# bababyVN/medical-image-segmentation-and-classification

Measured on AMD Instinct MI355X. Metric: images/sec (train step) Attention U-Net 256x256 bs=32/GPU, higher is better.
Workload: dtype bf16; 1 GPU; AttentionUNet 256x256 train step (fwd+BCE+bwd+clip+AdamW), bs=32/GPU, NHWC bf16 activations, fp32 master weights; global_batch=32, parallelism=dp1, hip_graph=False, wgrad_side_stream=True, plan_replay=C (mi355_plan_run)

## Files before the change

include/mi355conv.h:

```cpp
#ifndef MI355CONV_H_
#define MI355CONV_H_

#include <stdint.h>

#ifdef __cplusplus
extern "C" {
#endif

typedef struct ihipStream_t* mi355_stream_t;

enum { MI355_F32 = 0, MI355_BF16 = 1, MI355_F16 = 2 };
enum { MI355_OK = 0, MI355_ERR_ARG = -1, MI355_ERR_UNSUPPORTED = -2, MI355_ERR_RUNTIME = -3 };

int mi355_version(void);
const char* mi355_last_error(void);


int mi355_pack_input_nchw(const float* x, void* y, int N, int C, int H, int W, int Cpad, int dtype,
                          mi355_stream_t s);
int mi355_pack_input_im2col3(const float* x, void* y, int N, int C, int H, int W, int dtype, mi355_stream_t s);
int mi355_unpack_output_nchw(const void* x, float* y, int N, int C, int H, int W, int ld, int dtype,
                             mi355_stream_t s);
int mi355_pack_nchw(const float* x, void* y, int N, int C, int H, int W, int ld, int dtype, mi355_stream_t s);

int mi355_pack_conv_weight(const float* w, void* wf, void* wb, int Co, int Ci, int Cip, int KH, int KW,
                           int transposed, int dtype, mi355_stream_t s);

int mi355_pack_conv_weights_batched(const int64_t* table, int n, int fields ,
                                    int dtype, mi355_stream_t s);

int mi355_conv2d_igemm(const void* in, const void* wk, const float* bias, void* out,
                       int N, int Hi, int Wi, int Ci, int ldi,
                       int Ho, int Wo, int Co, int ldo,
                       int KH, int KW, int mul, int kmul, int off, int div, int up,
                       int accumulate, float* stats, int dtype, mi355_stream_t s);
int mi355_conv2d_igemm_variant(int Hi, int Wi, int Ci, int Ho, int Wo, int Co, int KH, int KW, int mul, int kmul, int off,
                               int div, int up, int dtype);
int mi355_conv2d_igemm_variant_n(int N, int Hi, int Wi, int Ci, int Ho, int Wo, int Co, int KH, int KW, int mul, int kmul,
                                 int off, int div, int up, int dtype);
int mi355_conv2d_igemm_dma_tile(int N, int Ho, int Wo, int Ci, int Co);
int mi355_conv2d_igemm_generic_tile(int N, int Ho, int Wo, int Co);
int mi355_conv2d_igemm_stat_rows(int N, int Hi, int Wi, int Ci, int Ho, int Wo, int Co, int KH, int KW,
                                 int mul, int kmul, int off, int div, int up, int dtype);

int mi355_conv2d_wgrad_splits(int N, int Ho, int Wo, int Ci, int Co, int KH, int KW);
int mi355_conv2d_wgrad_variant(int N, int Ho, int Wo, int KH, int KW, int stride, int pad, int dtype);
int mi355_conv2d_wgrad(const void* x, const void* dy, float* ws, int splits,
                       int N, int Hi, int Wi, int Ci, int ldx,
                       int Ho, int Wo, int Co, int ldy,
                       int KH, int KW, int stride, int pad, int up, int dtype, mi355_stream_t s);
int mi355_conv2d_wgrad_multi_ok(int N, int Ho, int Wo, int dtype);
int mi355_conv2d_wgrad_multi(const void* x0, const void* dy0, const void* x1, const void* dy1, const void* x2, const void* dy2,
                             const void* x3, const void* dy3, const void* x4, const void* dy4, const void* x5, const void* dy5,
                             int napp, float* ws, int splits, int N, int Hi, int Wi, int Ci, int ldx, int Ho, int Wo, int Co,
                             int ldy, int up, int dtype, mi355_stream_t s);
int mi355_conv2d_wgrad_reduce(const float* ws, int splits, float* dw, int Co, int Ci, int Ci_real,
                              int KH, int KW, int transposed, float beta, mi355_stream_t s);


int mi355_rowreduce_blocks(long long M);
int mi355_bn_stats(const void* x, float* partial, long long M, int C, int ld, int dtype, mi355_stream_t s);
int mi355_bn_finalize(const float* partial, int nblocks, long long M, int C, const float* gamma,
                      const float* beta, float* running_mean, float* running_var, int64_t* nbt,
                      float momentum, float eps, float* scale, float* shift, float* mean, float* invstd,
                      mi355_stream_t s);
int mi355_fold_rows(const float* partial, int rows, int rowlen, float* out, int nsplit, mi355_stream_t s);
int mi355_bn_fold_bias(const float* bias, const float* scale, const float* shift, float* out, int C, mi355_stream_t s);
int mi355_bn_eval_coeffs(const float* gamma, const float* beta, const float* running_mean,
                         const float* running_var, float eps, int C, float* scale, float* shift,
                         mi355_stream_t s);
int mi355_bn_act(const void* x, int ldx, const float* scale, const float* shift,
                 const void* x2, int ldx2, const float* scale2, const float* shift2,
                 const void* res, int ldr, void* y, int ldy, long long M, int C, int act, int dtype,
                 mi355_stream_t s);
int mi355_bn_act_pool2(const void* x, int ldx, const float* scale, const float* shift, void* y, int ldy, void* p, int ldp,
                       int N, int H, int W, int C, int act, int dtype, mi355_stream_t s);
int mi355_bn_act_windows(const void* x, int ldx, const float* scale, const float* shift, const void* res, int ldr, void* y, int ldy,
                         int N, int H, int W, int C, int act, int dtype, mi355_stream_t s);
int mi355_bn_bwd_reduce_rows(long long M);
int mi355_bn_bwd_reduce(const void* dy, int lddy, const void* y, int ldy, const void* x, int ldx,
                        const float* mean, const float* invstd, const float* mscale, const float* mshift,
                        float* partial, long long M, int C, int act, int dtype, mi355_stream_t s);
int mi355_bn_bwd_finalize(const float* partial, int nblocks, int C, float* sums, float* dgamma, float* dbeta,
                          float acc, mi355_stream_t s);
int mi355_bn_bwd_finalize_at(const float* partial, int nblocks, int nq, int q0, int q1, int C, float* sums, float* dgamma,
                             float* dbeta, float acc, mi355_stream_t s);
int mi355_bn_bwd_apply(const void* dy, int lddy, const void* y, int ldy, const void* x, int ldx,
                       const float* gamma, const float* mean, const float* invstd, const float* mscale,
                       const float* mshift, const float* sums, void* dx, int lddx, void* dres, int lddres,
                       void* dpost, int lddpost, int post_acc, float* dbias_partial,
                       long long M, int C, int act, int dtype, mi355_stream_t s);
int mi355_bn_bwd_apply_post4(const void* dy, int lddy, const void* y, int ldy, const void* x, int ldx,
                             const float* gamma, const float* mean, const float* invstd, const float* mscale,
                             const float* mshift, const float* sums, void* dx, int lddx, void* dpost, int lddpost,
                             int post_acc, const void* ex0, const void* ex1, const void* ex2, const void* ex3, int ldex,
                             long long M, int C, int act, int dtype, mi355_stream_t s);
int mi355_bn_bwd_pool2_ok(int H, int W, int C, int dtype);
int mi355_bn_bwd_reduce_pool2_rows(long long M);
int mi355_bn_bwd_reduce_pool2(const void* dy, int lddy, const void* dp, int lddp, const void* x, int ldx, const float* mean,
                              const float* invstd, const float* mscale, const float* mshift, float* partial,
                              int N, int H, int W, int C, int dtype, mi355_stream_t s);
int mi355_bn_bwd_apply_pool2(const void* dy, int lddy, const void* dp, int lddp, const void* x, int ldx, const float* gamma,
                             const float* mean, const float* invstd, const float* mscale, const float* mshift,
                             const float* sums, void* dx, int lddx, int N, int H, int W, int C, int dtype, mi355_stream_t s);
int mi355_colsum_finalize(const float* partial, int nblocks, int stride, int C, float* out, float acc,
                          mi355_stream_t s);
int mi355_colsum(const void* x, int ld, float* partial, long long M, int C, int dtype, mi355_stream_t s);

int mi355_maxpool_fwd(const void* x, int ldx, void* y, int ldy, int N, int H, int W, int C,
                      int k, int stride, int pad, int dtype, mi355_stream_t s);
int mi355_maxpool_bwd(const void* x, int ldx, const void* dy, int lddy, void* dx, int lddx,
                      int N, int H, int W, int C, int k, int stride, int pad, int accumulate, int dtype,
                      mi355_stream_t s);
int mi355_upsample2_bwd(const void* dy, int lddy, void* dx, int lddx, int N, int H, int W, int C,
                        int accumulate, int dtype, mi355_stream_t s);
int mi355_add(const void* a, int lda, const void* b, int ldb, void* y, int ldy, long long M, int C, int dtype,
              mi355_stream_t s);
int mi355_relu_fwd(const void* x, int ldx, void* y, int ldy, long long M, int C, int dtype, mi355_stream_t s);
int mi355_relu_bwd(const void* dy, int lddy, const void* y, int ldy, void* dx, int lddx, long long M, int C,
                   int dtype, mi355_stream_t s);

int mi355_rowdot_fwd(const void* x, int ldx, const float* w, const float* b, float* z, float* partial,
                     long long M, int C, int HW, int K, int dtype, mi355_stream_t s);
int mi355_rowdot_bwd(const float* dz, const void* x, int ldx, const float* w, void* dx, int lddx,
                     float* partial, long long M, int C, int relu_mask, int HW, int K, int accumulate, int dtype,
                     mi355_stream_t s);
int mi355_gate_mul_fwd(const void* x, int ldx, const float* z, const float* scale, const float* shift,
                       void* y, int ldy, long long M, int C, int dtype, mi355_stream_t s);
int mi355_gate_mul_bwd(const void* dy, int lddy, const void* x, int ldx, const float* z, const float* scale,
// ... 103 lines not shown
```

medical-image-segmentation-and-classification_amd/csrc/conv_wgrad.hip:

```cpp
#include "common.hpp"
#include "dma.hpp"
#include "wgrad3x3_halo.hpp"
#include "wgrad3x3_halo8.hpp"
#include <stdlib.h>

struct WgradArgs {
  const void* x;
  const void* dy;
  float* ws;
  int N, Hi, Wi, Ci, ldx;
  int Ho, Wo, Co, ldy;
  int KH, KW, stride, pad, up;
  int M, Hlog, Wlog;
  int chunk;
};

typedef __attribute__((address_space(3))) s16x4 lds_s16x4;
template <typename T> struct TwoByte { typedef T type; };
template <> struct TwoByte<float> { typedef bf16_t type; };

template <typename T, int BCO, int BCI>
__global__ __launch_bounds__(256) void conv_wgrad_kernel(const WgradArgs a) {
  constexpr int BP = 32;
  constexpr int EPC = 16 / (int)sizeof(T);
  constexpr bool BF = sizeof(T) == 2;
  constexpr int PO = BF ? (BCO == 128 ? 320 : 192) : BCO * 4;
  constexpr int PX = BF ? (BCI == 128 ? 320 : 192) : BCI * 4;
  constexpr int O_BYTES = BP * PO, X_BYTES = BP * PX, STAGE = O_BYTES + X_BYTES;
  constexpr int CPRO = BCO / EPC, CPRX = BCI / EPC;
  constexpr int O_IT = BP * CPRO / 256, X_IT = BP * CPRX / 256;
  constexpr int WTO = BCO / 2, WTI = BCI / 2;
  constexpr int MI = WTO / 32, NI = WTI / 32;
  static_assert(O_IT >= 1 && X_IT >= 1, "tile too small for 256 threads");
  __shared__ __attribute__((aligned(16))) unsigned char lds[2 * STAGE];

  const int tid = threadIdx.x, lane = tid & 63, wave = tid >> 6;
  const int r32 = lane & 31, h = lane >> 5;
  const int wo_ = wave >> 1, wi_ = wave & 1;
  const int ciTiles = (a.Ci + BCI - 1) / BCI;
  int bid = xcd_tile((blockIdx.z * gridDim.y + blockIdx.y) * gridDim.x + blockIdx.x, gridDim.x * gridDim.y * gridDim.z);
  const int bx = bid % gridDim.x; bid /= gridDim.x;
  const int co0 = (bx / ciTiles) * BCO, ci0 = (bx % ciTiles) * BCI;
  const int tap = bid % gridDim.y, kh = tap / a.KW, kw = tap - kh * a.KW;
  const int split = bid / gridDim.y;
  const int p_begin = split * a.chunk;
  const int p_end = min(a.M, p_begin + a.chunk);
  const T* __restrict__ x = reinterpret_cast<const T*>(a.x);
  const T* __restrict__ dy = reinterpret_cast<const T*>(a.dy);

  int o_row[O_IT], o_c[O_IT];
#pragma unroll
  for (int i = 0; i < O_IT; ++i) {
    const int id = tid + i * 256;
    o_row[i] = id / CPRO;
    o_c[i] = id - o_row[i] * CPRO;
  }
  int x_row[X_IT], x_c[X_IT], x_n[X_IT], x_ho[X_IT], x_wo[X_IT];
  const int HoWo = a.Ho * a.Wo;
#pragma unroll
  for (int i = 0; i < X_IT; ++i) {
    const int id = tid + i * 256;
    x_row[i] = id / CPRX;
    x_c[i] = id - x_row[i] * CPRX;
    const int m = p_begin + x_row[i];
    x_n[i] = m / HoWo;
    const int rem = m - x_n[i] * HoWo;
    x_ho[i] = rem / a.Wo;
    x_wo[i] = rem - x_ho[i] * a.Wo;
  }

  uint4 ro[O_IT], rx[X_IT];
  auto load_tile = [&](int p0) {
#pragma unroll
    for (int i = 0; i < O_IT; ++i) {
      const int m = p0 + o_row[i];
      const int c = co0 + o_c[i] * EPC;
      if (m < p_end && c < a.Co)
        ro[i] = *reinterpret_cast<const uint4*>(dy + (size_t)m * a.ldy + c);
      else
        ro[i] = make_uint4(0, 0, 0, 0);
    }
#pragma unroll
    for (int i = 0; i < X_IT; ++i) {
      const int m = p0 + x_row[i];
      const int c = ci0 + x_c[i] * EPC;
      int th = x_ho[i] * a.stride + kh - a.pad, tw = x_wo[i] * a.stride + kw - a.pad;
      bool ok = m < p_end && c < a.Ci && (unsigned)th < (unsigned)a.Hlog && (unsigned)tw < (unsigned)a.Wlog;
// ... 25 lines not shown
  f32x16 acc[MI][NI];
#pragma unroll
  for (int mi = 0; mi < MI; ++mi)
#pragma unroll
    for (int ni = 0; ni < NI; ++ni)
#pragma unroll
      for (int r = 0; r < 16; ++r) acc[mi][ni][r] = 0.f;

  const int steps = (p_end - p_begin + BP - 1) / BP;
  if (steps > 0) {
    load_tile(p_begin);
    store_tile(0);
  }
  __syncthreads();
  const int tq = (lane & 15) >> 2, tp = lane & 3, tg = (lane >> 4) & 1;
  for (int st = 0; st < steps; ++st) {
    const int cur = st & 1;
    const bool more = (st + 1) < steps;
    if (more) load_tile(p_begin + (st + 1) * BP);
    const unsigned char* lo = lds + cur * STAGE;
    const unsigned char* lx = lo + O_BYTES;
    if constexpr (BF) {
#pragma unroll
      for (int ss = 0; ss < 2; ++ss) {
        bf16x8 af[MI], bfr[NI];
#pragma unroll
        for (int mi = 0; mi < MI; ++mi) {
          const int col = wo_ * WTO + mi * 32 + 16 * tg + 4 * tp;
          const int prow = ss * 16 + 8 * h + tq;
          const s16x4 v0 = __builtin_amdgcn_ds_read_tr16_b64_v4i16((lds_s16x4*)(lo + prow * PO + col * 2));
          const s16x4 v1 = __builtin_amdgcn_ds_read_tr16_b64_v4i16((lds_s16x4*)(lo + (prow + 4) * PO + col * 2));
          af[mi] = __builtin_bit_cast(bf16x8, __builtin_shufflevector(v0, v1, 0, 1, 2, 3, 4, 5, 6, 7));
        }
#pragma unroll
        for (int ni = 0; ni < NI; ++ni) {
          const int col = wi_ * WTI + ni * 32 + 16 * tg + 4 * tp;
          const int prow = ss * 16 + 8 * h + tq;
          const s16x4 v0 = __builtin_amdgcn_ds_read_tr16_b64_v4i16((lds_s16x4*)(lx + prow * PX + col * 2));
          const s16x4 v1 = __builtin_amdgcn_ds_read_tr16_b64_v4i16((lds_s16x4*)(lx + (prow + 4) * PX + col * 2));
          bfr[ni] = __builtin_bit_cast(bf16x8, __builtin_shufflevector(v0, v1, 0, 1, 2, 3, 4, 5, 6, 7));
        }
#pragma unroll
        for (int mi = 0; mi < MI; ++mi)
#pragma unroll
          for (int ni = 0; ni < NI; ++ni)
            acc[mi][ni] = mfma_32x32x16<typename TwoByte<T>::type>(af[mi], bfr[ni], acc[mi][ni]);
      }
    } else {
#pragma unroll 4
      for (int s2 = 0; s2 < BP / 2; ++s2) {
        const int prow = 2 * s2 + h;
        float af[MI], bfr[NI];
#pragma unroll
        for (int mi = 0; mi < MI; ++mi)
          af[mi] = *reinterpret_cast<const float*>(lo + prow * PO + (wo_ * WTO + mi * 32 + r32) * 4);
#pragma unroll
        for (int ni = 0; ni < NI; ++ni)
          bfr[ni] = *reinterpret_cast<const float*>(lx + prow * PX + (wi_ * WTI + ni * 32 + r32) * 4);
#pragma unroll
        for (int mi = 0; mi < MI; ++mi)
#pragma unroll
          for (int ni = 0; ni < NI; ++ni)
            acc[mi][ni] = __builtin_amdgcn_mfma_f32_32x32x2f32(af[mi], bfr[ni], acc[mi][ni], 0, 0, 0);
      }
    }
    if (more) store_tile(cur ^ 1);
    __syncthreads();
  }

  const int taps = a.KH * a.KW;
  float* __restrict__ ws = a.ws + (size_t)split * a.Co * taps * a.Ci;
#pragma unroll
  for (int mi = 0; mi < MI; ++mi)
#pragma unroll
    for (int ni = 0; ni < NI; ++ni)
#pragma unroll
      for (int r = 0; r < 16; ++r) {
        const int co = co0 + wo_ * WTO + mi * 32 + (r & 3) + 8 * (r >> 2) + 4 * h;
        const int ci = ci0 + wi_ * WTI + ni * 32 + r32;
        if (co < a.Co && ci < a.Ci) ws[((size_t)co * taps + tap) * a.Ci + ci] = acc[mi][ni][r];
      }
}

static void wgrad_tiles(int Co, int Ci, int& bco, int& bci) {
  bco = (Co % 128 == 0) ? 128 : 64;
  bci = (Ci % 128 == 0) ? 128 : 64;
}

static int halo_wgrad_mode(int N, int Ho, int Wo, int KH, int KW) {
  static const int use8 = getenv("MI355_WGRAD8") ? atoi(getenv("MI355_WGRAD8")) : 1;
  if (KH != 3 || KW != 3 || Ho % 8 != 0) return 0;
  if (use8 && Wo % 64 == 0) return 3;
  if (use8 && Wo == 32 && N % 2 == 0) return 4;
  if (Wo % 32 == 0) return 1;
  if (Wo == 16 && N % 2 == 0) return 2;
  return 0;
}
static int halo_wgrad_items(int mode, int N, int Ho, int Wo, int rb) {
  switch (mode) {
    case 1: return N * (Wo / 32) * (Ho / rb);
    case 3: return N * (Wo / 64) * (Ho / rb);
    default: return (N / 2) * (Ho / rb);
  }
}

extern "C" int mi355_conv2d_wgrad_splits(int N, int Ho, int Wo, int Ci, int Co, int KH, int KW) {
  if (const int mode = halo_wgrad_mode(N, Ho, Wo, KH, KW)) {
    const int rb = Ho % 32 == 0 ? 32 : (Ho % 16 == 0 ? 16 : 8);
    const long long items = halo_wgrad_items(mode, N, Ho, Wo, rb);
    const long long tiles = (long long)ceil_div(Co, 64) * ceil_div(Ci, 64);
    static const int wgs_env = getenv("MI355_WGRAD_WGS") ? atoi(getenv("MI355_WGRAD_WGS")) : 0;
    int wgs = wgs_env > 0 ? wgs_env : (mode >= 3 ? 128 : 256);
    static const int deep_wgs = getenv("MI355_WGRAD_WGS_DEEP") ? atoi(getenv("MI355_WGRAD_WGS_DEEP")) : 0;
    static const int deep_h = getenv("MI355_WGRAD_DEEP_H") ? atoi(getenv("MI355_WGRAD_DEEP_H")) : 64;
    if (mode >= 3 && deep_wgs > 0 && Ho <= deep_h) wgs = deep_wgs;
    long long s = wgs / tiles;
    if (s > items) s = items;
    const long long slab = (long long)Co * 9 * Ci * 4;
    while (s > 1 && s * slab > (512ll << 20)) --s;
    return (int)(s < 1 ? 1 : s);
  }
  int bco, bci;
  wgrad_tiles(Co, Ci, bco, bci);
  const long long M = (long long)N * Ho * Wo;
  const long long tiles = (long long)ceil_div(Co, bco) * ceil_div(Ci, bci) * KH * KW;
  long long s = 768 / tiles;
  const long long max_by_pixels = M / 256 > 0 ? M / 256 : 1;
  if (s > max_by_pixels) s = max_by_pixels;
  const long long slab = (long long)Co * KH * KW * Ci * 4;
  while (s > 1 && s * slab > (512ll << 20)) --s;
  if (s < 1) s = 1;
  return (int)s;
}

template <typename T>
static int wgrad_launch(const WgradArgs& a, int splits, hipStream_t s) {
  int bco, bci;
  wgrad_tiles(a.Co, a.Ci, bco, bci);
  dim3 grid(ceil_div(a.Co, bco) * ceil_div(a.Ci, bci), a.KH * a.KW, splits);
  if (bco == 128 && bci == 128)
    hipLaunchKernelGGL((conv_wgrad_kernel<T, 128, 128>), grid, dim3(256), 0, s, a);
  else if (bco == 128)
    hipLaunchKernelGGL((conv_wgrad_kernel<T, 128, 64>), grid, dim3(256), 0, s, a);
  else if (bci == 128)
    hipLaunchKernelGGL((conv_wgrad_kernel<T, 64, 128>), grid, dim3(256), 0, s, a);
  else
    hipLaunchKernelGGL((conv_wgrad_kernel<T, 64, 64>), grid, dim3(256), 0, s, a);
  MI355_LAUNCH_CHECK();
  return MI355_OK;
}

template <typename T, bool W16>
static int launch_wgrad3x3(const Wgrad3Args& h, dim3 grid, hipStream_t s) {
  constexpr int lds_bytes = Wgrad3Lds<W16>::BYTES;
  static const hipError_t configured =
      hipFuncSetAttribute((const void*)wgrad3x3_halo_kernel<T, W16>, hipFuncAttributeMaxDynamicSharedMemorySize, lds_bytes);
  if (configured != hipSuccess)
    MI355_FAIL((int)configured, "wgrad3x3_halo: cannot reserve %d B of LDS: %s", lds_bytes, hipGetErrorString(configured));
  hipLaunchKernelGGL((wgrad3x3_halo_kernel<T, W16>), grid, dim3(256), lds_bytes, s, h);
  MI355_LAUNCH_CHECK();
  return MI355_OK;
}
template <typename T, bool W32>
static int launch_wgrad3x3_8(const Wgrad3Args& h, dim3 grid, hipStream_t s) {
  constexpr int lds_bytes = Wgrad8Lds::BYTES;
  static const hipError_t configured =
      hipFuncSetAttribute((const void*)wgrad3x3_halo8_kernel<T, W32>, hipFuncAttributeMaxDynamicSharedMemorySize, lds_bytes);
  if (configured != hipSuccess)
    MI355_FAIL((int)configured, "wgrad3x3_halo8: cannot reserve %d B of LDS: %s", lds_bytes, hipGetErrorString(configured));
  hipLaunchKernelGGL((wgrad3x3_halo8_kernel<T, W32>), grid, dim3(512), lds_bytes, s, h);
  MI355_LAUNCH_CHECK();
  return MI355_OK;
}
static int launch_wgrad3x3_any(const Wgrad3Args& h, dim3 grid, int hmode, int dtype, hipStream_t s) {
  const bool f16 = dtype == MI355_F16;
  switch (hmode) {
    case 2: return f16 ? launch_wgrad3x3<f16_t, true>(h, grid, s) : launch_wgrad3x3<bf16_t, true>(h, grid, s);
    case 3: return f16 ? launch_wgrad3x3_8<f16_t, false>(h, grid, s) : launch_wgrad3x3_8<bf16_t, false>(h, grid, s);
    case 4: return f16 ? launch_wgrad3x3_8<f16_t, true>(h, grid, s) : launch_wgrad3x3_8<bf16_t, true>(h, grid, s);
    default: return f16 ? launch_wgrad3x3<f16_t, false>(h, grid, s) : launch_wgrad3x3<bf16_t, false>(h, grid, s);
  }
}

extern "C" int mi355_conv2d_wgrad(const void* x, const void* dy, float* ws, int splits, int N, int Hi, int Wi, int Ci,
                                  int ldx, int Ho, int Wo, int Co, int ldy, int KH, int KW, int stride, int pad, int up,
                                  int dtype, mi355_stream_t s) {
  MI355_CHECK_ARG(x && dy && ws, "conv2d_wgrad: null pointer");
  MI355_CHECK_ARG(splits >= 1 && splits <= 65535, "conv2d_wgrad: splits=%d out of range", splits);
  const int esz = dtype_is_2byte(dtype) ? 2 : 4;
  const int epc = 16 / esz;
  MI355_CHECK_ARG(Ci % epc == 0 && Co % epc == 0, "conv2d_wgrad: Ci=%d / Co=%d must be multiples of %d", Ci, Co, epc);
  MI355_CHECK_ARG(((uintptr_t)x % 16) == 0 && ((uintptr_t)dy % 16) == 0 && (ldx * esz) % 16 == 0 && (ldy * esz) % 16 == 0,
                  "conv2d_wgrad: pointers / channel strides must be 16-byte aligned");
  MI355_CHECK_ARG((long long)N * Ho * Wo < (1ll << 31) && (long long)N * Hi * Wi < (1ll << 31),
                  "conv2d_wgrad: pixel count overflows int32");
  WgradArgs a;
  a.x = x; a.dy = dy; a.ws = ws;
  a.N = N; a.Hi = Hi; a.Wi = Wi; a.Ci = Ci; a.ldx = ldx;
  a.Ho = Ho; a.Wo = Wo; a.Co = Co; a.ldy = ldy;
  a.KH = KH; a.KW = KW; a.stride = stride; a.pad = pad; a.up = up ? 1 : 0;
  a.M = N * Ho * Wo;
  a.Hlog = up ? 2 * Hi : Hi;
  a.Wlog = up ? 2 * Wi : Wi;
  a.chunk = ceil_div(ceil_div(a.M, splits), 32) * 32;
  static const int use_halo = getenv("MI355_WGRAD_HALO") ? atoi(getenv("MI355_WGRAD_HALO")) : 1;
  const int hmode = halo_wgrad_mode(N, Ho, Wo, KH, KW);
  const long long img_lim = (1ll << 31) / (hmode == 2 || hmode == 4 ? 2 : 1);
  const bool fits = (long long)Hi * Wi * ldx * esz < img_lim && (long long)Ho * Wo * ldy * esz < img_lim;
  if (dtype_is_2byte(dtype) && use_halo && stride == 1 && pad == 1 && hmode && Ho == a.Hlog && Wo == a.Wlog && fits) {
    Wgrad3Args h;
    for (int i = 0; i < 6; ++i) { h.xs[i] = x; h.dys[i] = dy; }
    h.ws = ws;
    h.N = N; h.Hi = Hi; h.Wi = Wi; h.Ci = Ci; h.ldx = ldx;
    h.H = Ho; h.W = Wo; h.Co = Co; h.ldy = ldy; h.up = up ? 1 : 0;
    h.RB = Ho % 32 == 0 ? 32 : (Ho % 16 == 0 ? 16 : 8);
    h.items = halo_wgrad_items(hmode, N, Ho, Wo, h.RB);
    h.items_per_app = h.items;
    h.items_per_block = ceil_div(h.items, splits);
    dim3 grid(ceil_div(Co, 64) * ceil_div(Ci, 64), splits);
    return launch_wgrad3x3_any(h, grid, hmode, dtype, (hipStream_t)s);
  }
  return dispatch_dtype(dtype, "conv2d_wgrad", [&](auto tag) { return wgrad_launch<decltype(tag)>(a, splits, (hipStream_t)s); });
}

extern "C" int mi355_conv2d_wgrad_variant(int N, int Ho, int Wo, int KH, int KW, int stride, int pad, int dtype) {
  static const int use_halo = getenv("MI355_WGRAD_HALO") ? atoi(getenv("MI355_WGRAD_HALO")) : 1;
  if (!use_halo || !dtype_is_2byte(dtype) || stride != 1 || pad != 1) return 0;
  return halo_wgrad_mode(N, Ho, Wo, KH, KW);
}

extern "C" int mi355_conv2d_wgrad_multi_ok(int N, int Ho, int Wo, int dtype) {
  static const int use_halo = getenv("MI355_WGRAD_HALO") ? atoi(getenv("MI355_WGRAD_HALO")) : 1;
  return (use_halo && dtype_is_2byte(dtype) && halo_wgrad_mode(N, Ho, Wo, 3, 3)) ? 1 : 0;
}

extern "C" int mi355_conv2d_wgrad_multi(const void* x0, const void* dy0, const void* x1, const void* dy1, const void* x2,
                                        const void* dy2, const void* x3, const void* dy3, const void* x4, const void* dy4,
                                        const void* x5, const void* dy5, int napp, float* ws, int splits, int N, int Hi, int Wi,
                                        int Ci, int ldx, int Ho, int Wo, int Co, int ldy, int up, int dtype, mi355_stream_t s) {
  const void* xs[6] = {x0, x1, x2, x3, x4, x5};
  const void* dys[6] = {dy0, dy1, dy2, dy3, dy4, dy5};
  MI355_CHECK_ARG(napp >= 1 && napp <= 6 && ws && splits >= 1, "conv2d_wgrad_multi: 1..6 operand pairs, a workspace, splits >= 1");
  for (int i = 0; i < napp; ++i)
    MI355_CHECK_ARG(xs[i] && dys[i] && ((uintptr_t)xs[i] % 16) == 0 && ((uintptr_t)dys[i] % 16) == 0,
                    "conv2d_wgrad_multi: pair %d: null or misaligned pointer", i);
  MI355_CHECK_ARG(mi355_conv2d_wgrad_multi_ok(N, Ho, Wo, dtype), "conv2d_wgrad_multi: shape / dtype not served by the nine-tap kernel "
                  "(mi355_conv2d_wgrad_multi_ok == 0): run mi355_conv2d_wgrad per pair");
  MI355_CHECK_ARG(Ci % 8 == 0 && Co % 8 == 0 && (ldx * 2) % 16 == 0 && (ldy * 2) % 16 == 0 && ldx >= Ci && ldy >= Co,
                  "conv2d_wgrad_multi: channel counts / strides must be multiples of 8 elements");
  MI355_CHECK_ARG((up ? (Ho == 2 * Hi && Wo == 2 * Wi) : (Ho == Hi && Wo == Wi)), "conv2d_wgrad_multi: 3x3 / stride 1 / pad 1 geometry only");
  MI355_CHECK_ARG((long long)Hi * Wi * ldx * 4 < (1ll << 31) && (long long)Ho * Wo * ldy * 4 < (1ll << 31),
                  "conv2d_wgrad_multi: an image of 1 GiB or more is beyond the 32-bit offsets of the nine-tap kernel's buffer descriptors");
  const int hmode = halo_wgrad_mode(N, Ho, Wo, 3, 3);
  Wgrad3Args h;
  for (int i = 0; i < 6; ++i) { h.xs[i] = xs[i < napp ? i : 0]; h.dys[i] = dys[i < napp ? i : 0]; }
  h.ws = ws;
  h.N = N; h.Hi = Hi; h.Wi = Wi; h.Ci = Ci; h.ldx = ldx;
  h.H = Ho; h.W = Wo; h.Co = Co; h.ldy = ldy; h.up = up ? 1 : 0;
  h.RB = Ho % 32 == 0 ? 32 : (Ho % 16 == 0 ? 16 : 8);
  h.items_per_app = halo_wgrad_items(hmode, N, Ho, Wo, h.RB);
  h.items = napp * h.items_per_app;
  MI355_CHECK_ARG(splits <= h.items, "conv2d_wgrad_multi: more splits (%d) than work items (%d)", splits, h.items);
  h.items_per_block = ceil_div(h.items, splits);
  dim3 grid(ceil_div(Co, 64) * ceil_div(Ci, 64), splits);
  return launch_wgrad3x3_any(h, grid, hmode, dtype, (hipStream_t)s);
}


#define WR_CI 32
template <int TAPS>
__global__ __launch_bounds__(1024) void wgrad_reduce_kernel(const float* __restrict__ ws, int splits, float* __restrict__ dw, int Co,
                                                            int Ci, int Ci_real, int taps_rt, int transposed, float beta, int KL) {
  extern __shared__ float tile[];
  const int taps = TAPS > 0 ? TAPS : taps_rt;
  const int ciTiles = (Ci + WR_CI - 1) / WR_CI;
  const int co = blockIdx.x / ciTiles, ci0 = (blockIdx.x % ciTiles) * WR_CI;
  const size_t total = (size_t)Co * taps * Ci;
  const int cl = threadIdx.x % WR_CI, kl = threadIdx.x / WR_CI;
  const int ci = ci0 + cl;
  const int tstride = taps * (WR_CI + 1);
  if constexpr (TAPS > 0) {
    float s0[TAPS], s1[TAPS];
#pragma unroll
    for (int tap = 0; tap < TAPS; ++tap) { s0[tap] = 0.f; s1[tap] = 0.f; }
    if (ci < Ci) {
      const float* p = ws + (size_t)co * TAPS * Ci + ci;
      int k = kl;
      for (; k + KL < splits; k += 2 * KL) {
        float a[TAPS], b[TAPS];
#pragma unroll
        for (int tap = 0; tap < TAPS; ++tap) {
          a[tap] = p[(size_t)k * total + (size_t)tap * Ci];
          b[tap] = p[(size_t)(k + KL) * total + (size_t)tap * Ci];
        }
#pragma unroll
        for (int tap = 0; tap < TAPS; ++tap) { s0[tap] += a[tap]; s1[tap] += b[tap]; }
      }
      if (k < splits) {
#pragma unroll
        for (int tap = 0; tap < TAPS; ++tap) s0[tap] += p[(size_t)k * total + (size_t)tap * Ci];
      }
    }
#pragma unroll
    for (int tap = 0; tap < TAPS; ++tap) tile[kl * tstride + tap * (WR_CI + 1) + cl] = s0[tap] + s1[tap];
// ... 47 lines not shown
```

medical-image-segmentation-and-classification_amd/mi355/graph.py:

```python
from __future__ import annotations

import ctypes
import os
import struct
from typing import List, Optional

import torch
import torch.nn as nn

from .lib import lib, DTYPE_CODE

BN_EPS_DEFAULT = 1e-5
CPAD = 32
FUSE_POOL = os.environ.get("MI355_FUSE_POOL", "1") != "0"
FUSE_POOL_BWD = os.environ.get("MI355_FUSE_POOL_BWD", "1") != "0"
FUSE_GATE_BWD = os.environ.get("MI355_FUSE_GATE_BWD", "1") != "0"
FUSE_HEAD = os.environ.get("MI355_FUSE_HEAD", "1") != "0"
STEM_IM2COL = os.environ.get("MI355_STEM_IM2COL", "1") != "0"
SIDE_COLSUM = os.environ.get("MI355_SIDE_COLSUM", "1") != "0"
BN_ACT_WINDOWS = os.environ.get("MI355_BN_ACT_WINDOWS", "1") != "0"
STATIC_PACKS = os.environ.get("MI355_STATIC_PACKS", "1") != "0"
BN_ACT_WINDOWS_RES = os.environ.get("MI355_BN_ACT_WINDOWS_RES", "1") != "0"
FUSE_RESIDUAL = os.environ.get("MI355_FUSE_RESIDUAL", "1") != "0"
DEFER_POST = os.environ.get("MI355_DEFER_POST", "1") != "0"
# ... 468 lines not shown
        out = self.f32(N * C * H * W)
        self.fwd.append(Launch("mi355_unpack_output_nchw", t, out, N, C, H, W, t.ld, self.code))
        self.output = ("z", out, (N, C, H, W))
        if self.want_grad and t.needs_grad:
            self.dout = self.f32(N * C * H * W)

            def rule():
                if self.acc_flag(t):
                    raise NotImplementedError("tensor_output of an activation with other consumers")
                g = self.grad_of(t)
                self.bwd.append(Launch("mi355_pack_nchw", self.dout, g, N, C, H, W, g.ld, self.code))
            self.rule(rule)
        return out

    def packs(self, conv, cip, transposed=False, scale=None):
        key = (id(conv), cip, id(scale))
        if key not in self._packs:
            w = conv.weight
            if transposed:
                ci, co = w.shape[0], w.shape[1]
            else:
                co, ci = w.shape[0], w.shape[1]
            k = w.shape[2]
            if hasattr(conv, "pack_shape"):
                co, ci, k = conv.pack_shape
            wf = self._alloc(co * k * k * cip)
            wb = self._alloc(co * k * k * cip) if self.want_grad else None
            assert k * k <= 288, "batched weight pack: at most 288 taps"
            self._pack_table.append((w, wf, wb, co, ci, cip, k * k, 1 if transposed else 0, scale))
            self.see(w, conv.bias)
            self._packs[key] = (wf, wb)
        return self._packs[key]

    def _conv_geom(self, x, conv, up):
        k, s, p = conv.kernel_size[0], conv.stride[0], conv.padding[0]
        if conv.kernel_size[0] != conv.kernel_size[1] or conv.dilation[0] != 1 or conv.groups != 1:
            raise NotImplementedError("square, undilated, ungrouped convolutions only")
        hl, wl = (2 * x.H, 2 * x.W) if up else (x.H, x.W)
        return k, s, p, (hl + 2 * p - k) // s + 1, (wl + 2 * p - k) // s + 1

    def conv_raw(self, x, conv, up=False, out=None, stats=False, relu=False, fold=None):
        stem = self._stem_as_pointwise(x, conv, up)
        if stem is not None:
            return self.conv_raw(stem[0], stem[1], out=out, stats=stats, relu=relu, fold=fold)
        if x is getattr(self, "_xin", None):
            self._xin_users += 1
        k, s, p, Ho, Wo = self._conv_geom(x, conv, up)
        Co = conv.out_channels
        assert x.C >= conv.in_channels and (x.C == conv.in_channels or conv.in_channels < CPAD), (x.C, conv.in_channels)
        wf, wb = self.packs(conv, x.C, scale=fold[0] if fold else None)
        bias = fold[1] if fold else conv.bias
        y = out if out is not None else self.new_tensor(x.N, Ho, Wo, Co)
        assert (y.N, y.H, y.W, y.C) == (x.N, Ho, Wo, Co)
        flops = 2 * x.N * Ho * Wo * Co * k * k * conv.in_channels
        nbytes = (x.N * x.H * x.W * x.C + x.N * Ho * Wo * Co + Co * k * k * x.C) * self.esz
        stat_part = None
        self._last_stat_rows = 0
        if stats and self.training:
            rows = lib.mi355_conv2d_igemm_stat_rows(x.N, x.H, x.W, x.C, Ho, Wo, Co, k, k, s, 1, -p, 1, 1 if up else 0, self.code)
            if rows > 0:
                stat_part = self.ws_f32(rows * 2 * Co)
                self._last_stat_rows = rows
        self.fwd.append(Launch("mi355_conv2d_igemm", x, wf, bias, y, x.N, x.H, x.W, x.C, x.ld, Ho, Wo, Co, y.ld,
                               k, k, s, 1, -p, 1, 1 if up else 0, 2 if relu else 0, stat_part, self.code, flops=flops, nbytes=nbytes,
                               tag=self.igemm_tag(x.N, x.H, x.W, x.C, Ho, Wo, Co, k, s, 1, -p, 1, 1 if up else 0)))
        y.needs_grad = x.needs_grad or self.param_grad(conv.weight)
        self._conv_uses[id(conv)] = self._conv_uses.get(id(conv), 0) + 1

        def bwd(dy, bias_done=False):
            uses = self._conv_uses[id(conv)]
            if (self.param_grad(conv.weight) and 1 < uses <= 6 and self.multi_wgrad and k == 3 and s == 1 and p == 1 and self.esz == 2
                    and lib.mi355_conv2d_wgrad_multi_ok(x.N, Ho, Wo, self.code)):
                pend = self._pending_wgrad.setdefault(id(conv), [])
                pend.append((x, dy))
                assert (x.N, x.H, x.W, x.C, x.ld, dy.ld) == tuple(getattr(pend[0][0], f) for f in ("N", "H", "W", "C", "ld")) + (pend[0][1].ld,)
                if len(pend) == uses:
                    self._emit_multi_wgrad(conv, pend, Ho, Wo, Co, k, up, flops, nbytes)
                    del self._pending_wgrad[id(conv)]
            elif self.param_grad(conv.weight):
                splits = lib.mi355_conv2d_wgrad_splits(x.N, Ho, Wo, x.C, Co, k, k)
                ws = self.ws_bytes(splits * Co * k * k * x.C * 4)
                self.bwd.append(Launch("mi355_conv2d_wgrad", x, dy, ws, splits, x.N, x.H, x.W, x.C, x.ld, Ho, Wo, Co, dy.ld,
                                       k, k, s, p, 1 if up else 0, self.code, flops=flops, nbytes=nbytes, side=True,
                                       tag=self.wgrad_tag(Co, x.C, k, s, Ho, Wo, x.N, p), cus=self.wgrad_cus(x.N, Ho, Wo, x.C, Co, k, s, p, splits)))
                ref, beta = self.pgrad(conv.weight)
                self.bwd.append(Launch("mi355_conv2d_wgrad_reduce", ws, splits, ref, Co, x.C, conv.in_channels, k, k, 0, beta, side=True))
            if conv.bias is not None and self.param_grad(conv.bias) and not bias_done:
                self.bias_grad_from(dy, conv.bias)
            if x.needs_grad:
                if up:
                    acc = self.acc_flag(x)
                    xg = self.grad_of(x)
                    tag = self.igemm_tag(x.N, Ho, Wo, Co, 2 * x.H, 2 * x.W, x.C, k, 1, -1, p, s, 0)
                    if lib.mi355_conv2d_igemm_variant_n(x.N, Ho, Wo, Co, 2 * x.H, 2 * x.W, x.C, k, k, 1, -1, p, s, 0, self.code) in (2, 3, 5, 6, 7, 8):
                        self.bwd.append(Launch("mi355_conv2d_igemm", dy, wb, None, xg, x.N, Ho, Wo, Co, dy.ld, 2 * x.H, 2 * x.W,
                                               x.C, xg.ld, k, k, 1, -1, p, s, 0, 4 | (1 if acc else 0), None, self.code, flops=flops,
                                               nbytes=nbytes, tag=tag))
                    else:
                        tmp = self.new_tensor(x.N, 2 * x.H, 2 * x.W, x.C)
                        self.bwd.append(Launch("mi355_conv2d_igemm", dy, wb, None, tmp, x.N, Ho, Wo, Co, dy.ld, 2 * x.H, 2 * x.W,
                                               x.C, tmp.ld, k, k, 1, -1, p, s, 0, 0, None, self.code, flops=flops, nbytes=nbytes, tag=tag))
                        self.bwd.append(Launch("mi355_upsample2_bwd", tmp, tmp.ld, xg, xg.ld, x.N, x.H, x.W, x.C, acc, self.code))
                else:
                    acc = self.acc_flag(x)
                    xg = self.grad_of(x)
                    self.bwd.append(Launch("mi355_conv2d_igemm", dy, wb, None, xg, x.N, Ho, Wo, Co, dy.ld, x.H, x.W, x.C,
                                           xg.ld, k, k, 1, -1, p, s, 0, acc, None, self.code, flops=flops, nbytes=nbytes,
                                           tag=self.igemm_tag(x.N, Ho, Wo, Co, x.H, x.W, x.C, k, 1, -1, p, s, 0)))
        return y, bwd

    def _emit_multi_wgrad(self, conv, pend, Ho, Wo, Co, k, up, flops, nbytes):
        x0 = pend[0][0]
        n = len(pend)
        splits = lib.mi355_conv2d_wgrad_splits(x0.N * n, Ho, Wo, x0.C, Co, k, k)
        ws = self.ws_bytes(splits * Co * k * k * x0.C * 4)
        ops = []
        for i in range(6):
            ops += list(pend[i]) if i < n else [None, None]
        self.bwd.append(Launch("mi355_conv2d_wgrad_multi", *ops, n, ws, splits, x0.N, x0.H, x0.W, x0.C, x0.ld, Ho, Wo, Co,
                               pend[0][1].ld, 1 if up else 0, self.code, flops=flops * n, nbytes=nbytes * n, side=True,
                               tag=self.wgrad_tag(Co, x0.C, k, 1, Ho, Wo, x0.N, 1), cus=self.wgrad_cus(x0.N, Ho, Wo, x0.C, Co, k, 1, 1, splits)))
        ref, beta = self.pgrad(conv.weight)
        self.bwd.append(Launch("mi355_conv2d_wgrad_reduce", ws, splits, ref, Co, x0.C, conv.in_channels, k, k, 0, beta, side=True))

    def igemm_tag(self, N, Hi, Wi, ci, Ho, Wo, co, k, mul, kmul, off, div, up):
        bn = 128 if co % 128 == 0 else (64 if co % 64 == 0 else 32)
        if self.dtype == torch.float32:
            return f"conv_igemm_kernel<f32,{lib.mi355_conv2d_igemm_generic_tile(N, Ho, Wo, co)},16>"
        v = lib.mi355_conv2d_igemm_variant_n(N, Hi, Wi, ci, Ho, Wo, co, k, k, mul, kmul, off, div, up, self.code)
        k64 = ci % 64 == 0
        if v == 0:
            return f"conv_igemm_kernel<bf16,{lib.mi355_conv2d_igemm_generic_tile(N, Ho, Wo, co)},{64 if k64 else 32}>"
        if v == 1:
            bn = lib.mi355_conv2d_igemm_dma_tile(N, Ho, Wo, ci, co)
            if bn == 128:
                return "conv_igemm_dma_kernel<128,64,2>" if k64 else "conv_igemm_dma_kernel<128,32,3>"
            return "conv_igemm_dma_kernel<64,32,3>" if bn == 64 else "conv_igemm_dma_kernel<32,64,3>"
        return {2: "conv3x3_halo_rw_kernel<8,32>", 3: "conv3x3_halo_rw_kernel<16,16>", 4: f"conv1x1_stream_kernel<{ci},{co}>",
                5: "conv3x3_halo_pp_kernel", 6: "conv3x3_halo_pp128_kernel", 7: "conv3x3_ws_kernel<64,8>", 8: "conv3x3_ws_kernel<128,4>",
                9: "conv_gemm256_kernel"}[v]

    def wgrad_tag(self, co, ci, k=1, s=1, Ho=0, Wo=0, N=0, p=None):
        t = "f32" if self.dtype == torch.float32 else "bf16"
        v = lib.mi355_conv2d_wgrad_variant(N, Ho, Wo, k, k, s, (k // 2) if p is None else p, self.code) if t == "bf16" else 0
        if v:
            return "wgrad3x3_halo8_kernel" if v >= 3 else "wgrad3x3_halo_kernel"
        return f"conv_wgrad_kernel<{t},{128 if co % 128 == 0 else 64},{128 if ci % 128 == 0 else 64}>"

    def wgrad_cus(self, N, Ho, Wo, ci, co, k, s, p, splits):
        if self.esz != 2 or lib.mi355_conv2d_wgrad_variant(N, Ho, Wo, k, k, s, p, self.code) < 3:
            return 1.0
        return min(1.0, -(-co // 64) * -(-ci // 64) * splits / 256.0)

    def bias_grad_from(self, dy, bias):
        nb = lib.mi355_rowreduce_blocks(dy.M)
        part = self.ws_f32(nb * dy.C)
        self.bwd.append(Launch("mi355_colsum", dy, dy.ld, part, dy.M, dy.C, self.code))
        ref, beta = self.pgrad(bias)
        self.bwd.append(Launch("mi355_colsum_finalize", part, nb, 1, dy.C, ref, beta))

    def _bn_coeffs(self, y, bn, fused_rows=0):
        C = bn.num_features
        st = {k: self.f32(C) for k in ("scale", "shift", "mean", "invstd")}
        self.see(bn.weight, bn.bias)
        if self.training:
            if fused_rows > 0:
                nb = fused_rows
                part = self.ws_f32(nb * 2 * C)
                if nb > 2048:
                    folded = self.f32(64 * 2 * C)
                    self.fwd.append(Launch("mi355_fold_rows", part, nb, 2 * C, folded, 64))
                    part, nb = folded, 64
            else:
                nb = lib.mi355_rowreduce_blocks(y.M)
                part = self.ws_f32(nb * 2 * C)
                self.fwd.append(Launch("mi355_bn_stats", y, part, y.M, C, y.ld, self.code))
            mom = bn.momentum if bn.momentum is not None else 0.1
            track = bn.track_running_stats
            self.fwd.append(Launch("mi355_bn_finalize", part, nb, y.M, C, bn.weight, bn.bias,
                                   bn.running_mean if track else None, bn.running_var if track else None,
                                   bn.num_batches_tracked if track else None, float(mom), float(bn.eps),
                                   st["scale"], st["shift"], st["mean"], st["invstd"]))
        else:
            self.fwd.append(Launch("mi355_bn_eval_coeffs", bn.weight, bn.bias, bn.running_mean, bn.running_var, float(bn.eps),
                                   C, st["scale"], st["shift"]))
        return st

    def _bn_bwd(self, da, a, y, bn, st, act, dres_to=None, bias=None, post_to=None, pool_dp=None, head=None):
        C = bn.num_features
        nb = lib.mi355_rowreduce_blocks(y.M)
        part = self.ws_f32(nb * 2 * C)
        if head is not None:
            dz, hconv = head
            assert act and dres_to is None and post_to is None and pool_dp is None
            part = self.f32(nb * 5 * C) if SIDE_COLSUM else self.ws_f32(nb * 5 * C)
            co = (st["scale"], st["shift"], st["mean"], st["invstd"], None, None, None, None)
            self.bwd.append(Launch("mi355_gate_bn_bwd_reduce", dz, y, y.ld, None, 0, *co, hconv.weight, part, y.M, C, self.code,
                                   nbytes=y.M * C * self.esz + 4 * y.M))
            head_folds = []
            if self.param_grad(hconv.weight):
                wref, wbeta = self.pgrad(hconv.weight)
                head_folds.append(Launch("mi355_colsum_finalize", self._ws_off(part, 3 * C * 4), nb, 5, C, wref, wbeta, side=SIDE_COLSUM))
                if hconv.bias is not None:
                    bref2, bbeta = self.pgrad(hconv.bias)
                    head_folds.append(Launch("mi355_colsum_finalize", self._ws_off(part, 4 * C * 4), nb, 5 * C, 1, bref2, bbeta, side=SIDE_COLSUM))
            sums = self.f32(2 * C)
            need_pg = self.param_grad(bn.weight)
            if need_pg:
                gref, gbeta = self.pgrad(bn.weight)
                bref, _ = self.pgrad(bn.bias)
            self.bwd.append(Launch("mi355_bn_bwd_finalize_at", part, min(nb, lib.mi355_gate_bn_bwd_reduce_rows(y.M)), 5, 0, 1, C, sums,
                                   gref if need_pg else None, bref if need_pg else None, gbeta if need_pg else 0.0))
            if bias is not None and self.param_grad(bias) and id(bias) not in self._grad_first:
                self.pgrad(bias)
                self.zero_grad_params.append(bias)
            dy = self.grad_of(y)
            self.bwd.append(Launch("mi355_gate_bn_bwd_apply", dz, y, y.ld, None, 0, *co, hconv.weight, bn.weight, None, sums, None,
                                   dy, dy.ld, None, 0, y.M, C, self.code, nbytes=2 * y.M * C * self.esz + 4 * y.M))
            self.bwd += head_folds
            return dy
        if pool_dp is not None:
            assert act and dres_to is None and post_to is None
            dal = da.ld if da is not None else 0
            self.bwd.append(Launch("mi355_bn_bwd_reduce_pool2", da, dal, pool_dp, pool_dp.ld, y, y.ld, st["mean"], st["invstd"],
                                   st["scale"], st["shift"], part, y.N, y.H, y.W, C, self.code,
                                   nbytes=int((1.25 + (da is not None)) * y.M * C * self.esz)))
            sums = self.f32(2 * C)
            need_pg = self.param_grad(bn.weight)
            if need_pg:
                gref, gbeta = self.pgrad(bn.weight)
# ... 635 lines not shown
```

Baseline: 2131 images/s.

## Add specialized 1x1 pointwise wgrad kernel with register-prefetch pipeline

Adds a dedicated weight-gradient kernel for 1x1 stride-1 unpadded convolutions in bf16/fp16. It drops the tap dimension and the generic spatial index math, and prefetches four pixel tiles ahead in registers while double-buffering through LDS. Tiles are read with transposed LDS reads feeding MFMA. It is enabled by default through an env switch, and the Python tag logic is updated so the plan records the new kernel name. The cost is a larger register footprint from the deep prefetch, which may reduce occupancy.

New measurement: 2132 images/s, median of 5. No clear change (+0.1%).

```diff
diff --git a/include/mi355conv.h b/include/mi355conv.h
--- a/include/mi355conv.h
+++ b/include/mi355conv.h
@@ -45,6 +45,7 @@
 
 int mi355_conv2d_wgrad_splits(int N, int Ho, int Wo, int Ci, int Co, int KH, int KW);
 int mi355_conv2d_wgrad_variant(int N, int Ho, int Wo, int KH, int KW, int stride, int pad, int dtype);
+int mi355_conv2d_wgrad_pw(int KH, int KW, int stride, int pad, int up, int dtype);
 int mi355_conv2d_wgrad(const void* x, const void* dy, float* ws, int splits,
                        int N, int Hi, int Wi, int Ci, int ldx,
                        int Ho, int Wo, int Co, int ldy,
diff --git a/medical-image-segmentation-and-classification_amd/csrc/conv_wgrad.hip b/medical-image-segmentation-and-classification_amd/csrc/conv_wgrad.hip
--- a/medical-image-segmentation-and-classification_amd/csrc/conv_wgrad.hip
+++ b/medical-image-segmentation-and-classification_amd/csrc/conv_wgrad.hip
@@ -3,6 +3,7 @@
 #include "wgrad3x3_halo.hpp"
 #include "wgrad3x3_halo8.hpp"
 #include <stdlib.h>
+#include <type_traits>
 
 struct WgradArgs {
   const void* x;
@@ -194,6 +195,151 @@
       }
 }
 
+template <typename T, int BCO, int BCI, int DEPTH>
+__global__ __launch_bounds__(256) void conv_wgrad_pw_kernel(const WgradArgs a) {
+  static_assert(sizeof(T) == 2, "bf16 / fp16 only");
+  constexpr int BP = 32, EPC = 8;
+  constexpr int PO = BCO == 128 ? 320 : 192, PX = BCI == 128 ? 320 : 192;
+  constexpr int O_BYTES = BP * PO, X_BYTES = BP * PX, STAGE = O_BYTES + X_BYTES;
+  constexpr int CPRO = BCO / EPC, CPRX = BCI / EPC;
+  constexpr int O_IT = BP * CPRO / 256, X_IT = BP * CPRX / 256;
+  constexpr int WTO = BCO / 2, WTI = BCI / 2;
+  constexpr int MI = WTO / 32, NI = WTI / 32;
+  static_assert(O_IT >= 1 && X_IT >= 1, "tile too small for 256 threads");
+  __shared__ __attribute__((aligned(16))) unsigned char lds[2 * STAGE];
+
+  const int tid = threadIdx.x, lane = tid & 63, wave = tid >> 6;
+  const int r32 = lane & 31, h = lane >> 5;
+  const int wo_ = wave >> 1, wi_ = wave & 1;
+  const int ciTiles = (a.Ci + BCI - 1) / BCI;
+  int bid = xcd_tile((blockIdx.z * gridDim.y + blockIdx.y) * gridDim.x + blockIdx.x, gridDim.x * gridDim.y * gridDim.z);
+  const int bx = bid % gridDim.x; bid /= gridDim.x;
+  const int co0 = (bx / ciTiles) * BCO, ci0 = (bx % ciTiles) * BCI;
+  const int split = bid / gridDim.y;
+  const int p_begin = split * a.chunk;
+  const int p_end = min(a.M, p_begin + a.chunk);
+  const T* __restrict__ x = reinterpret_cast<const T*>(a.x);
+  const T* __restrict__ dy = reinterpret_cast<const T*>(a.dy);
+
+  int o_row[O_IT], o_c[O_IT], x_row[X_IT], x_c[X_IT];
+#pragma unroll
+  for (int i = 0; i < O_IT; ++i) { const int id = tid + i * 256; o_row[i] = id / CPRO; o_c[i] = id - o_row[i] * CPRO; }
+#pragma unroll
+  for (int i = 0; i < X_IT; ++i) { const int id = tid + i * 256; x_row[i] = id / CPRX; x_c[i] = id - x_row[i] * CPRX; }
+  bool o_cok[O_IT], x_cok[X_IT];
+  int o_cc[O_IT], x_cc[X_IT];
+#pragma unroll
+  for (int i = 0; i < O_IT; ++i) { const int c = co0 + o_c[i] * EPC; o_cok[i] = c < a.Co; o_cc[i] = o_cok[i] ? c : a.Co - EPC; }
+#pragma unroll
+  for (int i = 0; i < X_IT; ++i) { const int c = ci0 + x_c[i] * EPC; x_cok[i] = c < a.Ci; x_cc[i] = x_cok[i] ? c : a.Ci - EPC; }
+
+  uint4 ro[DEPTH][O_IT], rx[DEPTH][X_IT];
+  auto masked = [](uint4 v, bool ok) {
+    const unsigned k = ok ? ~0u : 0u;
+    return make_uint4(v.x & k, v.y & k, v.z & k, v.w & k);
+  };
+  auto load_tile = [&](auto set_tag, int p0) {
+    constexpr int set = decltype(set_tag)::value;
+#pragma unroll
+    for (int i = 0; i < O_IT; ++i) {
+      const int m = min(p0 + o_row[i], p_end - 1);
+      ro[set][i] = *reinterpret_cast<const uint4*>(dy + (size_t)m * a.ldy + o_cc[i]);
+    }
+#pragma unroll
+    for (int i = 0; i < X_IT; ++i) {
+      const int m = min(p0 + x_row[i], p_end - 1);
+      rx[set][i] = *reinterpret_cast<const uint4*>(x + (size_t)m * a.ldx + x_cc[i]);
+    }
+  };
+  auto store_tile = [&](auto set_tag, int p0, int stage) {
+    constexpr int set = decltype(set_tag)::value;
+    unsigned char* lo = lds + stage * STAGE;
+    unsigned char* lx = lo + O_BYTES;
+#pragma unroll
+    for (int i = 0; i < O_IT; ++i)
+      *reinterpret_cast<uint4*>(lo + o_row[i] * PO + o_c[i] * 16) = masked(ro[set][i], o_cok[i] && p0 + o_row[i] < p_end);
+#pragma unroll
+    for (int i = 0; i < X_IT; ++i)
+      *reinterpret_cast<uint4*>(lx + x_row[i] * PX + x_c[i] * 16) = masked(rx[set][i], x_cok[i] && p0 + x_row[i] < p_end);
+  };
+
+  f32x16 acc[MI][NI];
+#pragma unroll
+  for (int mi = 0; mi < MI; ++mi)
+#pragma unroll
+    for (int ni = 0; ni < NI; ++ni)
+#pragma unroll
+      for (int r = 0; r < 16; ++r) acc[mi][ni][r] = 0.f;
+
+  const int steps = (p_end - p_begin + BP - 1) / BP;
+  static_assert(DEPTH == 4, "four step bodies per trip");
+  using J0 = std::integral_constant<int, 0>;
+  using J1 = std::integral_constant<int, 1>;
+  using J2 = std::integral_constant<int, 2>;
+  using J3 = std::integral_constant<int, 3>;
+  load_tile(J0{}, p_begin);
+  load_tile(J1{}, p_begin + BP);
+  load_tile(J2{}, p_begin + 2 * BP);
+  load_tile(J3{}, p_begin + 3 * BP);
+  if (steps > 0) store_tile(J0{}, p_begin, 0);
+  __syncthreads();
+  const int tq = (lane & 15) >> 2, tp = lane & 3, tg = (lane >> 4) & 1;
+  auto step = [&](int st, auto jtag) {
+    constexpr int J = decltype(jtag)::value;
+    load_tile(jtag, p_begin + (st + DEPTH) * BP);
+    const unsigned char* lo = lds + (J & 1) * STAGE;
+    const unsigned char* lx = lo + O_BYTES;
+#pragma unroll
+    for (int ss = 0; ss < 2; ++ss) {
+      bf16x8 af[MI], bfr[NI];
+#pragma unroll
+      for (int mi = 0; mi < MI; ++mi) {
+        const int col = wo_ * WTO + mi * 32 + 16 * tg + 4 * tp;
+        const int prow = ss * 16 + 8 * h + tq;
+        const s16x4 v0 = __builtin_amdgcn_ds_read_tr16_b64_v4i16((lds_s16x4*)(lo + prow * PO + col * 2));
+        const s16x4 v1 = __builtin_amdgcn_ds_read_tr16_b64_v4i16((lds_s16x4*)(lo + (prow + 4) * PO + col * 2));
+        af[mi] = __builtin_bit_cast(bf16x8, __builtin_shufflevector(v0, v1, 0, 1, 2, 3, 4, 5, 6, 7));
+      }
+#pragma unroll
+      for (int ni = 0; ni < NI; ++ni) {
+        const int col = wi_ * WTI + ni * 32 + 16 * tg + 4 * tp;
+        const int prow = ss * 16 + 8 * h + tq;
+        const s16x4 v0 = __builtin_amdgcn_ds_read_tr16_b64_v4i16((lds_s16x4*)(lx + prow * PX + col * 2));
+        const s16x4 v1 = __builtin_amdgcn_ds_read_tr16_b64_v4i16((lds_s16x4*)(lx + (prow + 4) * PX + col * 2));
+        bfr[ni] = __builtin_bit_cast(bf16x8, __builtin_shufflevector(v0, v1, 0, 1, 2, 3, 4, 5, 6, 7));
+      }
+#pragma unroll
+      for (int mi = 0; mi < MI; ++mi)
+#pragma unroll
+        for (int ni = 0; ni < NI; ++ni) acc[mi][ni] = mfma_32x32x16<T>(af[mi], bfr[ni], acc[mi][ni]);
+    }
+    if (st + 1 < steps) store_tile(std::integral_constant<int, (J + 1) % DEPTH>{}, p_begin + (st + 1) * BP, (J + 1) & 1);
+    __syncthreads();
+  };
+  int st = 0;
+  for (; st + 4 <= steps; st += 4) {
+    step(st, J0{});
+    step(st + 1, J1{});
+    step(st + 2, J2{});
+    step(st + 3, J3{});
+  }
+  if (st < steps) step(st, J0{});
+  if (st + 1 < steps) step(st + 1, J1{});
+  if (st + 2 < steps) step(st + 2, J2{});
+
+  float* __restrict__ ws = a.ws + (size_t)split * a.Co * a.Ci;
+#pragma unroll
+  for (int mi = 0; mi < MI; ++mi)
+#pragma unroll
+    for (int ni = 0; ni < NI; ++ni)
+#pragma unroll
+      for (int r = 0; r < 16; ++r) {
+        const int co = co0 + wo_ * WTO + mi * 32 + (r & 3) + 8 * (r >> 2) + 4 * h;
+        const int ci = ci0 + wi_ * WTI + ni * 32 + r32;
+        if (co < a.Co && ci < a.Ci) ws[(size_t)co * a.Ci + ci] = acc[mi][ni][r];
+      }
+}
+
 static void wgrad_tiles(int Co, int Ci, int& bco, int& bci) {
   bco = (Co % 128 == 0) ? 128 : 64;
   bci = (Ci % 128 == 0) ? 128 : 64;
@@ -243,6 +389,33 @@
   while (s > 1 && s * slab > (512ll << 20)) --s;
   if (s < 1) s = 1;
   return (int)s;
+}
+
+static bool pw_wgrad(int KH, int KW, int stride, int pad, int up, int dtype) {
+  static const int use = getenv("MI355_WGRAD_PW") ? atoi(getenv("MI355_WGRAD_PW")) : 1;
+  return use && dtype_is_2byte(dtype) && KH == 1 && KW == 1 && stride == 1 && pad == 0 && !up;
+}
+
+extern "C" int mi355_conv2d_wgrad_pw(int KH, int KW, int stride, int pad, int up, int dtype) {
+  return pw_wgrad(KH, KW, stride, pad, up, dtype) ? 1 : 0;
+}
+
+template <typename T>
+static int wgrad_pw_launch(const WgradArgs& a, int splits, hipStream_t s) {
+  constexpr int D = 4;
+  int bco, bci;
+  wgrad_tiles(a.Co, a.Ci, bco, bci);
+  dim3 grid(ceil_div(a.Co, bco) * ceil_div(a.Ci, bci), 1, splits);
+  if (bco == 128 && bci == 128)
+    hipLaunchKernelGGL((conv_wgrad_pw_kernel<T, 128, 128, D>), grid, dim3(256), 0, s, a);
+  else if (bco == 128)
+    hipLaunchKernelGGL((conv_wgrad_pw_kernel<T, 128, 64, D>), grid, dim3(256), 0, s, a);
+  else if (bci == 128)
+    hipLaunchKernelGGL((conv_wgrad_pw_kernel<T, 64, 128, D>), grid, dim3(256), 0, s, a);
+  else
+    hipLaunchKernelGGL((conv_wgrad_pw_kernel<T, 64, 64, D>), grid, dim3(256), 0, s, a);
+  MI355_LAUNCH_CHECK();
+  return MI355_OK;
 }
 
 template <typename T>
@@ -332,6 +505,8 @@
     dim3 grid(ceil_div(Co, 64) * ceil_div(Ci, 64), splits);
     return launch_wgrad3x3_any(h, grid, hmode, dtype, (hipStream_t)s);
   }
+  if (pw_wgrad(KH, KW, stride, pad, up, dtype) && Hi == Ho && Wi == Wo)
+    return dtype == MI355_F16 ? wgrad_pw_launch<f16_t>(a, splits, (hipStream_t)s) : wgrad_pw_launch<bf16_t>(a, splits, (hipStream_t)s);
   return dispatch_dtype(dtype, "conv2d_wgrad", [&](auto tag) { return wgrad_launch<decltype(tag)>(a, splits, (hipStream_t)s); });
 }
 
diff --git a/medical-image-segmentation-and-classification_amd/mi355/graph.py b/medical-image-segmentation-and-classification_amd/mi355/graph.py
--- a/medical-image-segmentation-and-classification_amd/mi355/graph.py
+++ b/medical-image-segmentation-and-classification_amd/mi355/graph.py
@@ -574,7 +574,7 @@
                 ws = self.ws_bytes(splits * Co * k * k * x.C * 4)
                 self.bwd.append(Launch("mi355_conv2d_wgrad", x, dy, ws, splits, x.N, x.H, x.W, x.C, x.ld, Ho, Wo, Co, dy.ld,
                                        k, k, s, p, 1 if up else 0, self.code, flops=flops, nbytes=nbytes, side=True,
-                                       tag=self.wgrad_tag(Co, x.C, k, s, Ho, Wo, x.N, p), cus=self.wgrad_cus(x.N, Ho, Wo, x.C, Co, k, s, p, splits)))
+                                       tag=self.wgrad_tag(Co, x.C, k, s, Ho, Wo, x.N, p, up), cus=self.wgrad_cus(x.N, Ho, Wo, x.C, Co, k, s, p, splits)))
                 ref, beta = self.pgrad(conv.weight)
                 self.bwd.append(Launch("mi355_conv2d_wgrad_reduce", ws, splits, ref, Co, x.C, conv.in_channels, k, k, 0, beta, side=True))
             if conv.bias is not None and self.param_grad(conv.bias) and not bias_done:
@@ -632,12 +632,14 @@
                 5: "conv3x3_halo_pp_kernel", 6: "conv3x3_halo_pp128_kernel", 7: "conv3x3_ws_kernel<64,8>", 8: "conv3x3_ws_kernel<128,4>",
                 9: "conv_gemm256_kernel"}[v]
 
-    def wgrad_tag(self, co, ci, k=1, s=1, Ho=0, Wo=0, N=0, p=None):
+    def wgrad_tag(self, co, ci, k=1, s=1, Ho=0, Wo=0, N=0, p=None, up=False):
         t = "f32" if self.dtype == torch.float32 else "bf16"
-        v = lib.mi355_conv2d_wgrad_variant(N, Ho, Wo, k, k, s, (k // 2) if p is None else p, self.code) if t == "bf16" else 0
+        p = (k // 2) if p is None else p
+        v = lib.mi355_conv2d_wgrad_variant(N, Ho, Wo, k, k, s, p, self.code) if t == "bf16" else 0
         if v:
             return "wgrad3x3_halo8_kernel" if v >= 3 else "wgrad3x3_halo_kernel"
-        return f"conv_wgrad_kernel<{t},{128 if co % 128 == 0 else 64},{128 if ci % 128 == 0 else 64}>"
+        pw = t == "bf16" and lib.mi355_conv2d_wgrad_pw(k, k, s, p, 1 if up else 0, self.code)
+        return f"conv_wgrad{'_pw' if pw else ''}_kernel<{t},{128 if co % 128 == 0 else 64},{128 if ci % 128 == 0 else 64}>"
 
     def wgrad_cus(self, N, Ho, Wo, ci, co, k, s, p, splits):
         if self.esz != 2 or lib.mi355_conv2d_wgrad_variant(N, Ho, Wo, k, k, s, p, self.code) < 3:
```
